# druskus20/volym

Hardware: AMD Instinct MI355X
Metric: Mrays/s + achieved HBM GB/s, 256^3 uint8 @ 1920x1080 (higher is better)
Workload: dtype u8 voxels, f32 compositing

## Files before the change

volym_amd/csrc/raymarch_device.h:

```cpp
#pragma once

#include <hip/hip_runtime.h>

#include "wgsl_math.h"

namespace volym {

enum : uint32_t {
    F_CONE = 1u << 0,
    F_IMP_COLORING = 1u << 1,
    F_OPACITY = 1u << 2,
    F_IMP_RENDERING = 1u << 3,
    F_GAUSSIAN = 1u << 4,
    F_LINEAR = 1u << 5,
    F_WRITE_F32 = 1u << 6,
    F_RASTER = 1u << 7,
};

struct FrameParams {
    float ivp[16];
    float eye[3];
    float thr;
    float base_step;
    float min_step;
// ... 40 lines not shown
#define VOLYM_DF_IN_LDS(fp) (!VOLYM_DEV_SWITCHES || (fp).mc_n <= 32u)
#define VOLYM_DF_LDS_BYTES 16384

enum : uint32_t {
    CULL_CUBE_HULL = 1u << 0,
    CULL_OBJ_HULL = 1u << 1,
    CULL_AABB = 1u << 2,
    CULL_NOTHING_DENSE = 1u << 3,
    CULL_TILE_MASK = 1u << 4,
    CULL_TILE_DEPTH = 1u << 5,
};

struct FrameTables {
    float4 tf_tab[256];
    float4 lut_f[256];
    float ic_alpha[256];
    float rho[256];
};

struct Counters {
    unsigned long long n_vol, n_imp, n_steps, n_dense, n_hit;
};

struct V3 {
    float x, y, z;
};
__device__ __forceinline__ V3 v3(float x, float y, float z) { return V3{x, y, z}; }
__device__ __forceinline__ V3 operator+(V3 a, V3 b) { return v3(a.x + b.x, a.y + b.y, a.z + b.z); }
__device__ __forceinline__ V3 operator-(V3 a, V3 b) { return v3(a.x - b.x, a.y - b.y, a.z - b.z); }
__device__ __forceinline__ V3 operator*(V3 a, float s) { return v3(a.x * s, a.y * s, a.z * s); }
__device__ __forceinline__ V3 operator/(V3 a, float s) { return v3(a.x / s, a.y / s, a.z / s); }
__device__ __forceinline__ float dot_exact(V3 a, V3 b) { return (a.x * b.x + a.y * b.y) + a.z * b.z; }
__device__ __forceinline__ V3 cross(V3 a, V3 b)
{
    return v3(a.y * b.z - a.z * b.y, a.z * b.x - a.x * b.z, a.x * b.y - a.y * b.x);
}
__device__ __forceinline__ float length_exact(V3 a) { return __builtin_sqrtf(dot_exact(a, a)); }
__device__ __forceinline__ V3 normalize_exact(V3 a) { return a / length_exact(a); }
__device__ __forceinline__ float dot_fast(V3 a, V3 b)
{
    return __builtin_fmaf(a.z, b.z, __builtin_fmaf(a.y, b.y, a.x * b.x));
}

__host__ __device__ inline uint32_t brick_count(uint32_t n) { return (n + 3u) >> 2; }

template <bool BRICK>
// ... 510 lines not shown
    r.t_exit = __builtin_fmaxf(exit_, 0.0f);
    r.hit = !(r.t_exit <= r.t_entry);
}

__device__ __forceinline__ Ray make_ray_ieee(const FrameParams& fp, uint32_t gx, uint32_t gy)
{
    Ray r;
    const float scx = static_cast<float>(gx) / static_cast<float>(fp.W);
    const float scy = static_cast<float>(gy) / static_cast<float>(fp.H);
    const float ndx = scx * 2.0f - 1.0f;
    const float ndy = 1.0f - scy * 2.0f;
    float wp[4];
#pragma unroll
    for (int k = 0; k < 4; ++k)
        wp[k] = ((fp.ivp[k] * ndx + fp.ivp[4 + k] * ndy) + fp.ivp[8 + k] * 0.0f) + fp.ivp[12 + k] * 1.0f;
    r.o = v3(fp.eye[0], fp.eye[1], fp.eye[2]);
    const V3 world = v3(wp[0] / wp[3], wp[1] / wp[3], wp[2] / wp[3]);
    r.d = normalize_exact(world - r.o);
    ray_slabs(r, (0.0f - r.o.x) / r.d.x, (1.0f - r.o.x) / r.d.x, (0.0f - r.o.y) / r.d.y, (1.0f - r.o.y) / r.d.y,
              (0.0f - r.o.z) / r.d.z, (1.0f - r.o.z) / r.d.z);
    return r;
}

__device__ __forceinline__ Ray make_ray_shared(const FrameParams& fp, uint32_t gx, uint32_t gy, bool& ok)
{
    Ray r;
    const float scx = div_pixel(static_cast<float>(gx), static_cast<float>(fp.W), fp.rcp_w);
    const float scy = div_pixel(static_cast<float>(gy), static_cast<float>(fp.H), fp.rcp_h);
    const float ndx = scx * 2.0f - 1.0f;
    const float ndy = 1.0f - scy * 2.0f;
    float wp[4];
#pragma unroll
    for (int k = 0; k < 4; ++k)
        wp[k] = ((fp.ivp[k] * ndx + fp.ivp[4 + k] * ndy) + fp.ivp[8 + k] * 0.0f) + fp.ivp[12 + k] * 1.0f;
    r.o = v3(fp.eye[0], fp.eye[1], fp.eye[2]);
    const float rw = rcp_refined(wp[3]);
    const V3 a = v3(div_by(wp[0], wp[3], rw), div_by(wp[1], wp[3], rw), div_by(wp[2], wp[3], rw)) - r.o;
    const float len = length_exact(a);
    const float rl = rcp_refined(len);
    r.d = v3(div_by(a.x, len, rl), div_by(a.y, len, rl), div_by(a.z, len, rl));
    const float rx = rcp_refined(r.d.x), ry = rcp_refined(r.d.y), rz = rcp_refined(r.d.z);
    ray_slabs(r, div_by(0.0f - r.o.x, r.d.x, rx), div_by(1.0f - r.o.x, r.d.x, rx), div_by(0.0f - r.o.y, r.d.y, ry),
              div_by(1.0f - r.o.y, r.d.y, ry), div_by(0.0f - r.o.z, r.d.z, rz), div_by(1.0f - r.o.z, r.d.z, rz));
    const float lo = __builtin_fminf(__builtin_fminf(__builtin_fminf(__builtin_fabsf(wp[0]), __builtin_fabsf(wp[1])), __builtin_fabsf(wp[2])),
                                     __builtin_fminf(__builtin_fabsf(wp[3]), len));
    const float hi = __builtin_fmaxf(__builtin_fmaxf(__builtin_fmaxf(__builtin_fabsf(wp[0]), __builtin_fabsf(wp[1])), __builtin_fabsf(wp[2])),
                                     __builtin_fmaxf(__builtin_fabsf(wp[3]), len));
    const float dlo = __builtin_fminf(__builtin_fminf(__builtin_fabsf(r.d.x), __builtin_fabsf(r.d.y)), __builtin_fabsf(r.d.z));
    ok = lo > fp.setup_lo && hi < 0x1p+40f && dlo > 0x1p-30f;
    return r;
}

template <bool SHARED = true>
__device__ __forceinline__ Ray make_ray(const FrameParams& fp, uint32_t gx, uint32_t gy)
{
    if constexpr (!SHARED) return make_ray_ieee(fp, gx, gy);
    bool ok;
    const Ray r = make_ray_shared(fp, gx, gy, ok);
    if (__builtin_expect(__ballot(!ok) == 0ull, 1)) return r;
    return make_ray_ieee(fp, gx, gy);
}

}
```

volym_amd/csrc/raymarch_pq.h:

```cpp
#pragma once

#include <cstddef>
#include <type_traits>

#include "raymarch_device.h"
#include "worklist_entry.h"

namespace volym {

constexpr int PQ_WAVES = 16;
constexpr int PQ_WAVES_WIDE = 12;
constexpr uint32_t PQ_MIN_LEAP_D = 2;
constexpr int PQ_DP_DEPTH = 2;
constexpr int PQ_ITEMS_LDS = 512;
constexpr int pq_qcap(int k) { return 64 + 64 * k; }
constexpr float PQ_FIX_SCALE = 268435456.0f;
constexpr float PQ_FIX_INV = 1.0f / 268435456.0f;

__device__ __forceinline__ uint32_t lane_rank_in_mask(unsigned long long mask)
{
    return __builtin_amdgcn_mbcnt_hi(static_cast<uint32_t>(mask >> 32), __builtin_amdgcn_mbcnt_lo(static_cast<uint32_t>(mask), 0u));
}

typedef float f32x2 __attribute__((ext_vector_type(2)));
// ... 32 lines not shown
{
    const uint32_t bit = t8y * fp.mask_t8x + t8x;
    return ((fp.tile_mask[bit >> 5] >> (bit & 31u)) & 1u) != 0u;
}
struct PqKernelArgs {
    const uint8_t* vol; const uint8_t* imp; const FrameTables* tables; const uint8_t* df4; const uint2* order; uint32_t n_items; uint16_t* cost;
    uint32_t* out_shard; uint32_t* out_raster; float4* out_f32; Counters* counters; uint4* trace; FrameParams fp;
};
constexpr size_t PQ_FP_KERNARG_OFFSET = offsetof(PqKernelArgs, fp);
static_assert(PQ_FP_KERNARG_OFFSET % 8 == 0 && alignof(FrameParams) == 8, "FrameParams holds pointers: 8-byte aligned in the segment");

template <bool TABLE, bool COUNT, bool TRACE = false, int KSPEC = 1, bool IMP = true, bool BRICK = false, bool IR = false, int WAVES = PQ_WAVES, int CJ = 0, bool LB = false,
          bool RELOAD = true>
__global__ __launch_bounds__(WAVES * 64) void volym_raymarch_pq_kernel(
    const uint8_t* __restrict__ vol, const uint8_t* __restrict__ imp, const FrameTables* __restrict__ tables,
    const uint8_t* __restrict__ df4, const uint2* __restrict__ order, uint32_t n_items, uint16_t* __restrict__ cost,
    uint32_t* __restrict__ out_shard, uint32_t* __restrict__ out_raster, float4* __restrict__ out_f32,
    Counters* __restrict__ counters, uint4* __restrict__ trace, const FrameParams fp)
{
    constexpr int K = TABLE ? KSPEC : 2;
    constexpr int PQ_QCAP = pq_qcap(K);
    static_assert(K <= 4, "the shading queue of K > 4 does not fit the LDS");
    static_assert(CJ == 0 || IR, "look-ahead jobs belong to the importance-rendering instantiation");
    unsigned long long trace_t0 = 0;
    uint32_t trace_iters = 0, trace_flushes = 0, trace_tiles = 0, trace_marched = 0, trace_lanes = 0, trace_accepted = 0, trace_dp_iters = 0;
    unsigned long long tm_leap = 0, tm_samp = 0, tm_flush = 0, tm_mark = 0;
#define PQ_TICK() (TRACE ? __builtin_amdgcn_s_memtime() : 0ull)
    if (TRACE) trace_t0 = __builtin_amdgcn_s_memrealtime();

    __shared__ float4 s_tf_tab[256];
    __shared__ float4 s_lut[TABLE ? 1 : 256];
    __shared__ float s_ic_alpha[256];
    __shared__ float s_rho[256];
    __shared__ __attribute__((aligned(16))) uint8_t s_df[VOLYM_DF_LDS_BYTES];
    constexpr int THREADS = WAVES * 64;
    __shared__ float4 s_q[WAVES][PQ_QCAP];
    __shared__ uint32_t s_qm[WAVES][PQ_QCAP];
    __shared__ float s_qr[TABLE ? 1 : WAVES][TABLE ? 1 : PQ_QCAP];
    __shared__ uint32_t s_acc[WAVES][3][64];
    __shared__ float4 s_hh[WAVES][64];
    __shared__ uint8_t s_mail[(IMP || IR) ? WAVES : 1][(IMP || IR) ? 256 : 1];
    uint8_t (*const s_cres)[(IMP || IR) ? 256 : 1] = s_mail;
    constexpr uint32_t CJ_LPR = CJ == 2 ? 1u : 8u;
    constexpr uint32_t CJ_RPS = 64u / CJ_LPR;
    constexpr uint32_t CJ_CAP = CJ == 2 ? 64u : 32u;
    static_assert(!LB || (TABLE && BRICK && !IMP && !IR && !COUNT && K == 4), "LDS brick staging: bricked layout, common instantiation");
// ... 345 lines not shown
                        const size_t o = static_cast<size_t>(gy) * fe.W + gx;
                        out_raster[o] = packed;
                        if (flags & F_WRITE_F32) out_f32[o] = make_float4(0.0f, 0.0f, 0.0f, tclass == TILE_FILL_MISS ? 1.0f : 0.0f);
                    }
                } else {
                    out_shard[static_cast<size_t>(local_tile) * 256u + sub * 64u + sub_lane] = in_frame ? packed : 0u;
                }
                continue;
            }
        }
        if (TRACE) trace_marched++;

        acc_r[lane] = 0u; acc_g[lane] = 0u; acc_b[lane] = 0u;
        uint32_t q_head = 0, q_count = 0;

        Ray ray;
        ray.o = v3(0.0f, 0.0f, 0.0f); ray.d = v3(0.0f, 0.0f, 0.0f); ray.t_entry = 0.0f; ray.t_exit = 0.0f;
        ray.hit = false;
        if (in_frame) ray = make_ray<TABLE && !IMP && !IR>(fe, gx, gy);
        {
            const V3 hvec = ray_half_vector(ray.d);
            hh[lane] = make_float4(hvec.x, hvec.y, hvec.z, 0.0f);
        }
        bool active = in_frame && ray.hit;
        if (COUNT && active) n_hit++;
        float t = active ? ray.t_entry : 0.0f, cur = base, acc_a = active ? 0.0f : 1.0f;
        bool last_dense = false;
        if (culling && tclass == TILE_HIT_TEST) active = false;
        float t_end = ray.t_exit;
        if (culling && (fe.cull & CULL_AABB) && active) {
            const float rx = __builtin_amdgcn_rcpf(ray.d.x), ry = __builtin_amdgcn_rcpf(ray.d.y), rz = __builtin_amdgcn_rcpf(ray.d.z);
            const float ax0 = (fe.aabb_lo[0] - ray.o.x) * rx, ax1 = (fe.aabb_hi[0] - ray.o.x) * rx;
            const float ay0 = (fe.aabb_lo[1] - ray.o.y) * ry, ay1 = (fe.aabb_hi[1] - ray.o.y) * ry;
            const float az0 = (fe.aabb_lo[2] - ray.o.z) * rz, az1 = (fe.aabb_hi[2] - ray.o.z) * rz;
            float tn = __builtin_fmaxf(__builtin_fmaxf(__builtin_fminf(ax0, ax1), __builtin_fminf(ay0, ay1)), __builtin_fminf(az0, az1));
            float tf = __builtin_fminf(__builtin_fminf(__builtin_fmaxf(ax0, ax1), __builtin_fmaxf(ay0, ay1)), __builtin_fmaxf(az0, az1));
            tn = tn - 2.0e-5f * __builtin_fabsf(tn) - 1.0e-6f;
            tf = tf + 2.0e-5f * __builtin_fabsf(tf) + 1.0e-6f;
            if (fe.cull & CULL_TILE_DEPTH) {
                const auto* td = (const __attribute__((address_space(4))) uint32_t*)fe.tile_depth;
                const uint32_t t8 = (ty * 2u + (sub >> 1)) * fe.mask_t8x + tx * 2u + (sub & 1u);
                tn = __builtin_fmaxf(tn, __uint_as_float(~td[t8]));
                tf = __builtin_fminf(tf, __uint_as_float(td[32u * fe.mask_words + t8]));
            }
            const bool outside_static = (ray.d.x == 0.0f && (ray.o.x < fe.aabb_lo[0] || ray.o.x > fe.aabb_hi[0])) ||
                                        (ray.d.y == 0.0f && (ray.o.y < fe.aabb_lo[1] || ray.o.y > fe.aabb_hi[1])) ||
                                        (ray.d.z == 0.0f && (ray.o.z < fe.aabb_lo[2] || ray.o.z > fe.aabb_hi[2]));
            if (outside_static || !(tn <= tf)) {
                active = false;
            } else {
                t_end = __builtin_fminf(t_end, tf);
                const float t_first = __builtin_fminf(tn, t_end);
// ... 43 lines not shown
                    grad = v3(static_cast<float>(bxp - bxm), static_cast<float>(byp - bym), static_cast<float>(bzp - bzm));
                } else {
                    grad = v3(sample_density(g, s_rho, linear, v3(pos.x + o, pos.y, pos.z)) -
                                  sample_density(g, s_rho, linear, v3(pos.x - o, pos.y, pos.z)),
                              sample_density(g, s_rho, linear, v3(pos.x, pos.y + o, pos.z)) -
                                  sample_density(g, s_rho, linear, v3(pos.x, pos.y - o, pos.z)),
                              sample_density(g, s_rho, linear, v3(pos.x, pos.y, pos.z + o)) -
                                  sample_density(g, s_rho, linear, v3(pos.x, pos.y, pos.z - o)));
                }
                const float4 hv = hh[owner];
                const V3 shaded = blinn_phong_h(color, grad, v3(hv.x, hv.y, hv.z));
                atomicAdd(&acc_r[owner], static_cast<uint32_t>(__builtin_fmaf(shaded.x * w, PQ_FIX_SCALE, 0.5f)));
                atomicAdd(&acc_g[owner], static_cast<uint32_t>(__builtin_fmaf(shaded.y * w, PQ_FIX_SCALE, 0.5f)));
                atomicAdd(&acc_b[owner], static_cast<uint32_t>(__builtin_fmaf(shaded.z * w, PQ_FIX_SCALE, 0.5f)));
            }
            q_head += n;
            if (q_head >= PQ_QCAP) q_head -= PQ_QCAP;
            q_count -= n;
            __builtin_amdgcn_fence(__ATOMIC_SEQ_CST, "wavefront");
            __builtin_amdgcn_wave_barrier();
            if (TRACE) tm_flush += PQ_TICK() - fl0;
        };

        auto append = [&](bool emit, V3 p, float w, uint32_t meta, float rho) __attribute__((always_inline)) {
            if (VOLYM_DEV_SWITCHES && (fp.dev & 128u)) return;
            const unsigned long long mask = __ballot(emit);
            if (mask == 0ull) return;
            if (emit) {
                const uint32_t e0 = q_head + q_count + lane_rank_in_mask(mask), e = min(e0, e0 - PQ_QCAP);
                q4[e] = make_float4(p.x, p.y, p.z, w); qm[e] = meta;
                if (!TABLE) qr[e] = rho;
            }
            q_count += static_cast<uint32_t>(__popcll(mask));
            if (!TABLE && q_count >= 64u) flush(64u);
        };
        auto drain = [&]() __attribute__((always_inline)) { while (q_count >= 64u) flush(64u); };

        if (VOLYM_DEV_SWITCHES && (fp.dev & 256u)) active = false;
        if (TRACE) tm_mark = PQ_TICK();
        bool leap_ok = true;
        auto leap_phase = [&]() __attribute__((always_inline)) {
            active = active && t < t_end && acc_a < 0.95f;
            const bool want_leap = active && !last_dense && leap_ok;
            if (__ballot(want_leap) != 0ull) {
                const V3 pos = ray.o + ray.d * t;
                const float cxf = __builtin_floorf(pos.x * mcf), cyf = __builtin_floorf(pos.y * mcf), czf = __builtin_floorf(pos.z * mcf);
                const int cx = static_cast<int>(cxf), cy = static_cast<int>(cyf), cz = static_cast<int>(czf);
                const bool in_range = static_cast<uint32_t>(cx | cy | cz) < fp.mc_n;
                const uint32_t ci = in_range ? mad_u24(mad_u24(static_cast<uint32_t>(cz), fp.mc_n, static_cast<uint32_t>(cy)), fp.mc_n, static_cast<uint32_t>(cx)) : 0u;
                uint32_t D = (static_cast<uint32_t>(VOLYM_DF_IN_LDS(fp) ? s_df[ci >> 1] : df4[ci >> 1]) >> ((ci & 1u) * 4u)) & 15u;
                if (!(want_leap && in_range)) D = 0u;
                if (D >= PQ_MIN_LEAP_D) {
                    const float eps = gauss ? 4.0e-5f + 0.0101f : 4.0e-5f;
                    const float a = static_cast<float>(D - 1u) * inv_mc - eps;
                    const float lx = __builtin_fmaf(cxf, inv_mc, -a), hx = __builtin_fmaf(cxf, inv_mc, a + inv_mc);
                    const float ly = __builtin_fmaf(cyf, inv_mc, -a), hy = __builtin_fmaf(cyf, inv_mc, a + inv_mc);
                    const float lz = __builtin_fmaf(czf, inv_mc, -a), hz = __builtin_fmaf(czf, inv_mc, a + inv_mc);
                    const float ex = __builtin_fmaxf(__builtin_fmaf(lx, idx_, nox), __builtin_fmaf(hx, idx_, nox));
                    const float ey = __builtin_fmaxf(__builtin_fmaf(ly, idy_, noy), __builtin_fmaf(hy, idy_, noy));
                    const float ez = __builtin_fmaxf(__builtin_fmaf(lz, idz_, noz), __builtin_fmaf(hz, idz_, noz));
                    float te = __builtin_fminf(__builtin_fminf(ex, ey), ez);
                    te = te - 2.0e-5f * __builtin_fabsf(te);
                    const float t_stop = __builtin_fminf(te, t_end);
                    if (!COUNT) {
                        while (cur < base && t < t_stop) {
                            cur = __builtin_fminf(base, cur * 1.5f);
                            t += cur;
                        }
                        tile_trips++;
                        replay_saturated(t, t_stop, base);
                    }
                    while (COUNT && t < t_stop) {
                        if (COUNT) {
                            n_steps++; n_imp++;
                            if (gauss) {
                                const V3 q = ray.o + ray.d * t;
                                for (int i = -2; i <= 2; ++i) if (!outside01(q + ray.d * (static_cast<float>(i) * 0.005f))) n_vol++;
                            } else {
                                n_vol++;
                            }
                        }
                        cur = __builtin_fminf(base, cur * 1.5f);
                        t += cur;
                    }
                    if (!(t < t_end)) active = false;
                }
            }

        };

        if (dp) {
            const uint32_t kq = lane & 3u, qsh = lane & 60u;
            if constexpr (!IMP) {
                constexpr int J = PQ_DP_DEPTH;
                bool try_leap = true;
                active = active && t < t_end;
                while (__ballot(active) != 0ull) {
                    tile_iters++;
                    if (TRACE) { trace_iters++; trace_dp_iters++; trace_lanes += static_cast<uint32_t>(__popcll(__ballot(active))); tm_mark = PQ_TICK(); }
                    if (try_leap && !(VOLYM_DEV_SWITCHES && (fp.dev & 2u))) leap_phase();
                    if (TRACE) { const unsigned long long now = PQ_TICK(); tm_leap += now - tm_mark; tm_mark = now; }
                    constexpr int N = 4 * J;
                    float ts[N], cb[N], my_t[J];
                    {
                        float tt = t, cc = cur;
#pragma unroll
                        for (int sidx = 0; sidx < N; ++sidx) {
                            ts[sidx] = tt; cb[sidx] = cc;
                            if ((sidx & 3) == 0) my_t[sidx >> 2] = tt;
                            else my_t[sidx >> 2] = kq == static_cast<uint32_t>(sidx & 3) ? tt : my_t[sidx >> 2];
                            cc = last_dense ? min_step : __builtin_fminf(base, cc * 1.5f);
                            tt += cc;
                        }
                    }
                    V3 my_pos[J];
                    uint32_t my_b[J], my_ib[J];
#pragma unroll
                    for (int j = 0; j < J; ++j) {
                        my_ib[j] = 255u;
                        my_pos[j] = ray.o + ray.d * my_t[j];
                        const uint32_t off_j = nearest_offset(g, my_pos[j]);
                        my_b[j] = vol[off_j];
                        if (IR) my_ib[j] = imp[off_j];
                    }
                    drain();
                    uint32_t cm = 0;
                    float a4[J][4];
#pragma unroll
                    for (int j = 0; j < J; ++j) {
                        cm |= (static_cast<uint32_t>(__ballot(my_b[j] >= fp.thr_byte) >> qsh) & 15u) << (4 * j);
                        const int a_bits = __float_as_int(s_tf_tab[my_b[j]].w);
                        a4[j][0] = __int_as_float(__builtin_amdgcn_mov_dpp(a_bits, 0x00, 0xf, 0xf, true));
                        a4[j][1] = __int_as_float(__builtin_amdgcn_mov_dpp(a_bits, 0x55, 0xf, 0xf, true));
                        a4[j][2] = __int_as_float(__builtin_amdgcn_mov_dpp(a_bits, 0xaa, 0xf, 0xf, true));
                        a4[j][3] = __int_as_float(__builtin_amdgcn_mov_dpp(a_bits, 0xff, 0xf, 0xf, true));
                    }
                    uint32_t sm = 0;
                    if (IR) {
                        bool need[J], ahead[J];
#pragma unroll
                        for (int j = 0; j < J; ++j) { need[j] = active && my_b[j] >= fp.thr_byte && my_ib[j] < 255u; ahead[j] = false; }
                        if constexpr (CJ != 0) {
                            cj_lookahead(need, my_t, ray.o, ray.d, ray.t_exit, ahead);
                        } else if (flags & F_CONE) {
#pragma unroll
                            for (int j = 0; j < J; ++j)
                                ahead[j] = ahead_cone_wave(g, fp_here(), need[j], my_pos[j], ray.d, ray.t_exit, lane, fp.cone_cos[lane & 7u] * 0.2f, fp.cone_sin[lane & 7u] * 0.2f);
                        } else {
                            bool any_need = false;
#pragma unroll
                            for (int j = 0; j < J; ++j) any_need = any_need || need[j];
                            if (__ballot(any_need) != 0ull) ahead_straight_wave<J>(g, fp_here(), need, my_t, ray.o, ray.d, ray.t_exit, lane, mail, ahead, &la_rounds);
                        }
#pragma unroll
                        for (int j = 0; j < J; ++j) sm |= (static_cast<uint32_t>(__ballot(need[j] && ahead[j]) >> qsh) & 15u) << (4 * j);
                    }
                    uint32_t n_t = 0, n_a = 0;
                    float a_run = acc_a, a_after[N], my_w[J];
#pragma unroll
                    for (int sidx = 0; sidx < N; ++sidx) {
                        n_t += ts[sidx] < t_end ? 1u : 0u;
                        n_a += a_run < 0.95f ? 1u : 0u;
                        const float w = (1.0f - a_run) * a4[sidx >> 2][sidx & 3];
                        if ((sidx & 3) == 0) my_w[sidx >> 2] = w;
                        else my_w[sidx >> 2] = kq == static_cast<uint32_t>(sidx & 3) ? w : my_w[sidx >> 2];
                        a_run = (((cm & ~sm) >> sidx) & 1u) ? a_run + w : a_run;
                        a_after[sidx] = a_run;
                    }
                    const uint32_t full = (1u << N) - 1u;
                    const uint32_t mism = cm ^ (last_dense ? full : 0u);
                    const uint32_t n_c = min(static_cast<uint32_t>(__builtin_ctz(mism | (1u << N))) + 1u, static_cast<uint32_t>(N));
                    const uint32_t n_acc = min(min(n_t, n_a), n_c);
                    const uint32_t em = active ? (cm & ~sm & ((1u << n_acc) - 1u)) : 0u;
                    bool my_emit[J];
#pragma unroll
                    for (int j = 0; j < J; ++j) my_emit[j] = ((em >> (4 * j + kq)) & 1u) != 0u;
                    if (TRACE && kq == 0u && active) trace_accepted += n_acc;
                    const uint32_t last = n_acc - 1u;
                    float t_sel = ts[0], cb_sel = cb[0], a_sel = a_after[0];
#pragma unroll
                    for (int sidx = 1; sidx < N; ++sidx) {
                        const bool ge = last >= static_cast<uint32_t>(sidx);
                        t_sel = ge ? ts[sidx] : t_sel; cb_sel = ge ? cb[sidx] : cb_sel; a_sel = ge ? a_after[sidx] : a_sel;
                    }
                    const bool dl = ((cm >> last) & 1u) != 0u;
                    const bool last_dense_before = last_dense;
                    const float cur_new = dl ? min_step : __builtin_fminf(base, cb_sel * 1.5f);
                    if (active) {
                        cur = cur_new;
                        t = t_sel + cur_new;
                        acc_a = a_sel;
                        last_dense = dl;
                    }
                    leap_ok = !dl && !last_dense_before && n_acc == static_cast<uint32_t>(N);
                    try_leap = __ballot(active && leap_ok) != 0ull;
                    active = active && t < t_end && acc_a < 0.95f;
#pragma unroll
                    for (int j = 0; j < J; ++j) append(my_emit[j], my_pos[j], my_w[j], own | (my_b[j] << 8), 0.0f);
                    if (TRACE) tm_samp += PQ_TICK() - tm_mark;
                }
            } else {
            const bool use_alpha_dp = imp_coloring || (flags & F_OPACITY) != 0u;
            while (__ballot(active) != 0ull) {
                tile_iters++;
                if (TRACE) { trace_iters++; trace_dp_iters++; trace_lanes += static_cast<uint32_t>(__popcll(__ballot(active))); tm_mark = PQ_TICK(); }
                leap_phase();
                if (TRACE) { const unsigned long long now = PQ_TICK(); tm_leap += now - tm_mark; tm_mark = now; }
                float ts4[4], cs4[4];
                {
                    float tt = t, cc = cur;
#pragma unroll
                    for (int j = 0; j < 4; ++j) {
                        ts4[j] = tt;
                        cc = last_dense ? min_step : __builtin_fminf(base, cc * 1.5f);
                        cs4[j] = cc;
                        tt += cc;
                    }
                }
                const float tk = kq == 0u ? ts4[0] : (kq == 1u ? ts4[1] : (kq == 2u ? ts4[2] : ts4[3]));
                const V3 pos = ray.o + ray.d * tk;
                const uint32_t off = nearest_offset(g, pos);
// ... 52 lines not shown
                                        alpha += w;
                                    } else {
                                        if (static_cast<uint32_t>(j) == kq) { my_w = 1.0f; my_emit = true; }
                                        alpha = 1.0f;
                                        done = true; finished = true;
                                    }
                                }
                                if (dj != last_dense) done = true;
                            }
                        }
                    }
                    if (TRACE && kq == 0u) trace_accepted += static_cast<uint32_t>(last + 1);
                    if (last >= 0) {
                        const bool dl = ((quad_d >> last) & 1u) != 0u;
                        const float cur_before = last == 0 ? cur : (last == 1 ? cs4[0] : (last == 2 ? cs4[1] : cs4[2]));
                        const float t_last = last == 0 ? ts4[0] : (last == 1 ? ts4[1] : (last == 2 ? ts4[2] : ts4[3]));
                        cur = dl ? min_step : __builtin_fminf(base, cur_before * 1.5f);
                        if (!(finished && !use_alpha_dp && dl)) t = t_last + cur;
                        last_dense = dl;
                    }
                    acc_a = alpha;
                    if (finished) active = false;
                }
                append(my_emit, pos, my_w, own | (b << 8) | (ib << 16), rho_k);
                if (TRACE) tm_samp += PQ_TICK() - tm_mark;
            }
            }
        } else {
        while (__ballot(active) != 0ull) {
            tile_iters++;
            if (TRACE) { trace_iters++; trace_lanes += static_cast<uint32_t>(__popcll(__ballot(active))); tm_mark = PQ_TICK(); if (active) trace_ray_iters++; }
            leap_phase();
            if (TRACE) { const unsigned long long now = PQ_TICK(); tm_leap += now - tm_mark; tm_mark = now; }
            float ts[K];
            uint32_t offs[K], bs[K], ibs[K];
            float rhos[K];
            uint32_t taps[K];
            {
                float tt = t, cc = cur;
#pragma unroll
                for (int k = 0; k < K; ++k) {
                    ts[k] = tt;
                    cc = last_dense ? min_step : __builtin_fminf(base, cc * 1.5f);
                    tt += cc;
                }
                if constexpr (K % 2 == 0) {
#pragma unroll
                    for (int k = 0; k < K; k += 2) {
                        const f32x2 tp = {ts[k], ts[k + 1]};
                        const f32x2 ux = (ray.o.x + ray.d.x * tp) * g.fnx, uy = (ray.o.y + ray.d.y * tp) * g.fny, uz = (ray.o.z + ray.d.z * tp) * g.fnz;
                        offs[k] = voxel_offset(g, clamp_texel(floor_to_int(ux.x), static_cast<int>(g.hix)), clamp_texel(floor_to_int(uy.x), static_cast<int>(g.hiy)),
                                               clamp_texel(floor_to_int(uz.x), static_cast<int>(g.hiz)));
                        offs[k + 1] = voxel_offset(g, clamp_texel(floor_to_int(ux.y), static_cast<int>(g.hix)), clamp_texel(floor_to_int(uy.y), static_cast<int>(g.hiy)),
                                                   clamp_texel(floor_to_int(uz.y), static_cast<int>(g.hiz)));
                    }
                } else {
#pragma unroll
                    for (int k = 0; k < K; ++k) offs[k] = nearest_offset(g, ray.o + ray.d * ts[k]);
                }
#pragma unroll
                for (int k = 0; k < K; ++k) {
                    bs[k] = 0; ibs[k] = 0; rhos[k] = 0.0f; taps[k] = 1;
                    if (TABLE && !LB) bs[k] = vol[offs[k]];
                    if (IR) ibs[k] = imp[offs[k]];
                    if (active) {
                        if (!IR && need_imp) ibs[k] = imp[offs[k]];
                        if (!TABLE) {
                            const V3 p = ray.o + ray.d * ts[k];
                            uint32_t cnt = 0;
                            if (gauss) rhos[k] = sample_density_smoothed<true>(g, s_rho, linear, fp, p, ray.d, cnt);
                            else { rhos[k] = sample_density(g, s_rho, linear, p); cnt = 1; }
                            taps[k] = cnt;
                        }
                    }
                }
            }

            uint32_t lb_slots = 0xffffffffu;
            uint32_t lb_ld[2] = {0u, 0u}, lb_dst = 0xffffu;
            if constexpr (LB) {
                const uint32_t* const vol32 = reinterpret_cast<const uint32_t*>(vol);
                const unsigned long long act = __ballot(active);
                uint32_t used = 0u, n_new = 0u, lb_b[2] = {0u, 0u};
#pragma unroll
                for (int k = 0; k < K; ++k) {
                    const uint32_t bk = offs[k] >> 6;
                    unsigned long long todo = act;
                    while (todo != 0ull) {
                        const uint32_t b = __builtin_amdgcn_readlane(bk, __builtin_ctzll(todo));
                        const unsigned long long same = __ballot(bk == b) & todo;
                        todo &= ~same;
                        const uint32_t hit = static_cast<uint32_t>(__ballot(lb_tag == b)) & ((1u << LB_SLOTS) - 1u);
                        uint32_t sl;
                        if (hit != 0u) {
                            sl = static_cast<uint32_t>(__builtin_ctz(hit));
                            if (VOLYM_DEV_SWITCHES && (fp.dev & 512u) && lane == 0u) atomicAdd(&counters->n_hit, 1ull);
                        } else {
                            const uint32_t free_places = ~used & ((1u << LB_SLOTS) - 1u);
                            if (free_places == 0u || n_new == 8u) {
                                if (VOLYM_DEV_SWITCHES && (fp.dev & 512u) && lane == 0u) atomicAdd(&counters->n_dense, 1ull);
                                continue;
                            }
                            const uint32_t from_next = free_places & ~((1u << lb_next) - 1u);
                            sl = static_cast<uint32_t>(__builtin_ctz(from_next != 0u ? from_next : free_places));
                            lb_next = (sl + 1u) & (LB_SLOTS - 1u);
// ... 14 lines not shown
                if ((lb_dst >> 8) != 0xffu) lb_ld[1] = vol32[lb_b[1] * 16u + (lane & 15u)];
#pragma unroll
                for (int k = 0; k < K; ++k)
                    if (active && ((lb_slots >> (8 * k)) & 0xffu) == 0xffu) bs[k] = vol[offs[k]];
            }

            if (TABLE) drain();
            if constexpr (LB) {
                uint32_t* const lbw = s_lb[wave];
                if ((lb_dst & 0xffu) != 0xffu) lbw[(lb_dst & 0xffu) * 16u + (lane & 15u)] = lb_ld[0];
                if ((lb_dst >> 8) != 0xffu) lbw[(lb_dst >> 8) * 16u + (lane & 15u)] = lb_ld[1];
                const uint8_t* const lbb = reinterpret_cast<const uint8_t*>(lbw);
#pragma unroll
                for (int k = 0; k < K; ++k) {
                    const uint32_t sl = (lb_slots >> (8 * k)) & 0xffu;
                    if (sl != 0xffu) bs[k] = lbb[sl * 64u + (offs[k] & 63u)];
                }
            }

            if constexpr (TABLE && !COUNT && !IMP) {
                float a_tab[K];
#pragma unroll
                for (int k = 0; k < K; ++k) a_tab[k] = s_tf_tab[bs[k]].w;
                const bool predicted = last_dense;
                bool supp[K];
#pragma unroll
                for (int k = 0; k < K; ++k) supp[k] = false;
                if (IR) {
                    bool need[K];
                    bool chain = active;
#pragma unroll
                    for (int k = 0; k < K; ++k) {
                        const bool dense_k = bs[k] >= fp.thr_byte;
                        need[k] = chain && dense_k && ibs[k] < 255u;
                        chain = chain && dense_k == predicted;
                    }
                    if constexpr (CJ != 0) {
                        cj_lookahead(need, ts, ray.o, ray.d, ray.t_exit, supp);
                    } else if (flags & F_CONE) {
#pragma unroll
                        for (int k = 0; k < K; ++k)
                            supp[k] = ahead_cone_wave(g, fp_here(), need[k], ray.o + ray.d * ts[k], ray.d, ray.t_exit, lane, fp.cone_cos[lane & 7u] * 0.2f, fp.cone_sin[lane & 7u] * 0.2f);
                    } else {
                        bool any_need = false;
#pragma unroll
                        for (int k = 0; k < K; ++k) any_need = any_need || need[k];
                        if (__ballot(any_need) != 0ull) ahead_straight_wave<K>(g, fp_here(), need, ts, ray.o, ray.d, ray.t_exit, lane, mail, supp, &la_rounds);
                    }
#pragma unroll
                    for (int k = 0; k < K; ++k) supp[k] = supp[k] && need[k];
                }
                bool valid = active;
#pragma unroll
                for (int k = 0; k < K; ++k) {
                    const bool go = valid && t < t_end && acc_a < 0.95f;
                    if (TRACE && go) trace_accepted++;
                    const bool dense = bs[k] >= fp.thr_byte;
                    const bool emit = go && dense && !supp[k];
                    const float w = (1.0f - acc_a) * a_tab[k];
                    const V3 pos = ray.o + ray.d * t;
                    acc_a = emit ? acc_a + w : acc_a;
                    const float cur_next = dense ? min_step : __builtin_fminf(base, cur * 1.5f);
                    cur = go ? cur_next : cur;
                    t = go ? t + cur_next : t;
                    last_dense = go ? dense : last_dense;
                    valid = go && dense == predicted;
                    if (k == K - 1) leap_ok = go && !dense && !predicted;
                    append(emit, pos, w, own | (bs[k] << 8), 0.0f);
                }
                active = active && t < t_end && acc_a < 0.95f;
                if (TRACE) tm_samp += PQ_TICK() - tm_mark;
                continue;
            }
            bool ahead_pre[K];
            constexpr bool PRE_AHEAD = IMP && !COUNT && K > 1;
            const bool pre_ahead = PRE_AHEAD && imp_rendering && !imp_coloring;
            if (PRE_AHEAD && pre_ahead && (flags & F_CONE)) {
                bool chain = active;
#pragma unroll
                for (int k = 0; k < K; ++k) {
                    const bool dense_k = TABLE ? bs[k] >= fp.thr_byte : rhos[k] >= thr;
                    const bool need_k = chain && dense_k && ibs[k] < 255u;
                    chain = chain && dense_k == last_dense;
                    ahead_pre[k] = ahead_cone_wave(g, fp_here(), need_k, ray.o + ray.d * ts[k], ray.d, ray.t_exit, lane, fp.cone_cos[lane & 7u] * 0.2f, fp.cone_sin[lane & 7u] * 0.2f);
                }
            } else if (PRE_AHEAD && pre_ahead) {
                bool need[K];
                bool chain = active;
#pragma unroll
                for (int k = 0; k < K; ++k) {
                    const bool dense_k = TABLE ? bs[k] >= fp.thr_byte : rhos[k] >= thr;
                    need[k] = chain && dense_k && ibs[k] < 255u;
                    chain = chain && dense_k == last_dense;
// ... 40 lines not shown
                                                              : ahead_straight<COUNT>(g, fp, pos, ray.d, ray.t_exit, n_imp);
                                suppressed = ibs[k] < 255u && ahead;
                            }
                            if (TABLE) alpha_step = s_tf_tab[bs[k]].w;
                            else alpha_step = 1.0f - wgsl_pow(1.0f - sample_tf(s_lut, fp.tf_n, rhos[k]).w, fp.alpha_y);
                        }
                        if (!suppressed) {
                            if (COUNT) n_vol += 6;
                            emit = true;
                            if (use_alpha) {
                                w = (1.0f - acc_a) * alpha_step;
                                acc_a += w;
                            } else {
                                w = 1.0f;
                                acc_a = 1.0f;
                                advance = false;
                                active = false;
                                valid = false;
                            }
                        }
                    }
                    if (advance) t += cur;
                }
                append(emit, pos, w, own | (bs[k] << 8) | (ibs[k] << 16), rhos[k]);
            }
            if (TRACE) tm_samp += PQ_TICK() - tm_mark;
        }
        }
        drain();
        if (q_count) flush(q_count);

        if (in_frame && (!dp || (lane & 3u) == 0u)) {
            const float out_r = static_cast<float>(acc_r[own]) * PQ_FIX_INV, out_g = static_cast<float>(acc_g[own]) * PQ_FIX_INV,
                        out_b = static_cast<float>(acc_b[own]) * PQ_FIX_INV;
            const uint32_t packed = pack_rgba8(out_r, out_g, out_b, acc_a);
            if (flags & F_RASTER) {
                const size_t o = static_cast<size_t>(gy) * fe.W + gx;
                out_raster[o] = packed;
                if (flags & F_WRITE_F32) out_f32[o] = TRACE ? make_float4(static_cast<float>(trace_ray_iters), static_cast<float>(tile_iters), out_b, acc_a) : make_float4(out_r, out_g, out_b, acc_a);
            } else {
                out_shard[static_cast<size_t>(local_tile) * 256u + sub * 64u + sub_lane] = packed;
            }
        } else if (!in_frame && !(flags & F_RASTER) && (!dp || (lane & 3u) == 0u)) {
            out_shard[static_cast<size_t>(local_tile) * 256u + sub * 64u + sub_lane] = 0u;
        }
#ifndef VOLYM_COST_FLUSH
#define VOLYM_COST_FLUSH 2u
// ... 59 lines not shown
```

Measured before the change: 87790.

## Carry ray-march lane state as wave-wide ballot masks instead of per-lane bools

Replaces per-lane boolean control state (active, last_dense, leap_ok, emit, suppression) with 64-bit wave lane masks built by ballot and read back through inverse ballot. Loop conditions and the queue append then use the mask directly, so the repeated ballots on loop exits and emit decisions go away and the state can sit in scalar registers. A MASKS specialisation is added for table-mode, uninstrumented, non-importance instantiations, including a mask-based AABB and tile-depth cull. It adds a parallel code path that must keep matching the bool semantics, and some mask updates now differ subtly, for example the first-step go check.

```diff
diff --git a/volym_amd/csrc/raymarch_device.h b/volym_amd/csrc/raymarch_device.h
--- a/volym_amd/csrc/raymarch_device.h
+++ b/volym_amd/csrc/raymarch_device.h
@@ -86,6 +86,10 @@
     unsigned long long n_vol, n_imp, n_steps, n_dense, n_hit;
 };
 
+typedef unsigned long long lanemask;
+__device__ __forceinline__ lanemask lanes_where(bool single_compare) { return __builtin_amdgcn_ballot_w64(single_compare); }
+__device__ __forceinline__ bool lane_of(lanemask m) { return __builtin_amdgcn_inverse_ballot_w64(m); }
+
 struct V3 {
     float x, y, z;
 };
@@ -642,7 +646,7 @@
     return r;
 }
 
-__device__ __forceinline__ Ray make_ray_shared(const FrameParams& fp, uint32_t gx, uint32_t gy, bool& ok)
+__device__ __forceinline__ Ray make_ray_shared(const FrameParams& fp, uint32_t gx, uint32_t gy, lanemask& m_ok)
 {
     Ray r;
     const float scx = div_pixel(static_cast<float>(gx), static_cast<float>(fp.W), fp.rcp_w);
@@ -667,7 +671,14 @@
     const float hi = __builtin_fmaxf(__builtin_fmaxf(__builtin_fmaxf(__builtin_fabsf(wp[0]), __builtin_fabsf(wp[1])), __builtin_fabsf(wp[2])),
                                      __builtin_fmaxf(__builtin_fabsf(wp[3]), len));
     const float dlo = __builtin_fminf(__builtin_fminf(__builtin_fabsf(r.d.x), __builtin_fabsf(r.d.y)), __builtin_fabsf(r.d.z));
-    ok = lo > fp.setup_lo && hi < 0x1p+40f && dlo > 0x1p-30f;
+    m_ok = lanes_where(lo > fp.setup_lo) & lanes_where(hi < 0x1p+40f) & lanes_where(dlo > 0x1p-30f);
+    return r;
+}
+__device__ __forceinline__ Ray make_ray_shared(const FrameParams& fp, uint32_t gx, uint32_t gy, bool& ok)
+{
+    lanemask m_ok;
+    const Ray r = make_ray_shared(fp, gx, gy, m_ok);
+    ok = lane_of(m_ok);
     return r;
 }
 
@@ -675,9 +686,9 @@
 __device__ __forceinline__ Ray make_ray(const FrameParams& fp, uint32_t gx, uint32_t gy)
 {
     if constexpr (!SHARED) return make_ray_ieee(fp, gx, gy);
-    bool ok;
-    const Ray r = make_ray_shared(fp, gx, gy, ok);
-    if (__builtin_expect(__ballot(!ok) == 0ull, 1)) return r;
+    lanemask m_ok;
+    const Ray r = make_ray_shared(fp, gx, gy, m_ok);
+    if (__builtin_expect((~m_ok & lanes_where(true)) == 0ull, 1)) return r;
     return make_ray_ieee(fp, gx, gy);
 }
 
diff --git a/volym_amd/csrc/raymarch_pq.h b/volym_amd/csrc/raymarch_pq.h
--- a/volym_amd/csrc/raymarch_pq.h
+++ b/volym_amd/csrc/raymarch_pq.h
@@ -78,6 +78,8 @@
     constexpr int PQ_QCAP = pq_qcap(K);
     static_assert(K <= 4, "the shading queue of K > 4 does not fit the LDS");
     static_assert(CJ == 0 || IR, "look-ahead jobs belong to the importance-rendering instantiation");
+    constexpr bool MASKS = TABLE && !COUNT && !IMP;
+    static_assert(IMP || MASKS, "the pinned-flag instantiations are table mode and uninstrumented");
     unsigned long long trace_t0 = 0;
     uint32_t trace_iters = 0, trace_flushes = 0, trace_tiles = 0, trace_marched = 0, trace_lanes = 0, trace_accepted = 0, trace_dp_iters = 0;
     unsigned long long tm_leap = 0, tm_samp = 0, tm_flush = 0, tm_mark = 0;
@@ -469,12 +471,41 @@
             const V3 hvec = ray_half_vector(ray.d);
             hh[lane] = make_float4(hvec.x, hvec.y, hvec.z, 0.0f);
         }
-        bool active = in_frame && ray.hit;
+        lanemask m_active = lanes_where(gx < fe.W) & lanes_where(gy < fe.H) & lanes_where(!(ray.t_exit <= ray.t_entry));
+        lanemask m_last = 0ull, m_leap_ok = ~0ull;
+        bool active = MASKS ? lane_of(m_active) : in_frame && ray.hit;
         if (COUNT && active) n_hit++;
         float t = active ? ray.t_entry : 0.0f, cur = base, acc_a = active ? 0.0f : 1.0f;
         bool last_dense = false;
-        if (culling && tclass == TILE_HIT_TEST) active = false;
+        if (culling && tclass == TILE_HIT_TEST) { active = false; m_active = 0ull; }
         float t_end = ray.t_exit;
+        if constexpr (MASKS) {
+            if (culling && (fe.cull & CULL_AABB) && m_active != 0ull) {
+                const float rx = __builtin_amdgcn_rcpf(ray.d.x), ry = __builtin_amdgcn_rcpf(ray.d.y), rz = __builtin_amdgcn_rcpf(ray.d.z);
+                const float ax0 = (fe.aabb_lo[0] - ray.o.x) * rx, ax1 = (fe.aabb_hi[0] - ray.o.x) * rx;
+                const float ay0 = (fe.aabb_lo[1] - ray.o.y) * ry, ay1 = (fe.aabb_hi[1] - ray.o.y) * ry;
+                const float az0 = (fe.aabb_lo[2] - ray.o.z) * rz, az1 = (fe.aabb_hi[2] - ray.o.z) * rz;
+                float tn = __builtin_fmaxf(__builtin_fmaxf(__builtin_fminf(ax0, ax1), __builtin_fminf(ay0, ay1)), __builtin_fminf(az0, az1));
+                float tf = __builtin_fminf(__builtin_fminf(__builtin_fmaxf(ax0, ax1), __builtin_fmaxf(ay0, ay1)), __builtin_fmaxf(az0, az1));
+                tn = tn - 2.0e-5f * __builtin_fabsf(tn) - 1.0e-6f;
+                tf = tf + 2.0e-5f * __builtin_fabsf(tf) + 1.0e-6f;
+                if (fe.cull & CULL_TILE_DEPTH) {
+                    const auto* td = (const __attribute__((address_space(4))) uint32_t*)fe.tile_depth;
+                    const uint32_t t8 = (ty * 2u + (sub >> 1)) * fe.mask_t8x + tx * 2u + (sub & 1u);
+                    tn = __builtin_fmaxf(tn, __uint_as_float(~td[t8]));
+                    tf = __builtin_fminf(tf, __uint_as_float(td[32u * fe.mask_words + t8]));
+                }
+                const lanemask m_static = (lanes_where(ray.d.x == 0.0f) & (lanes_where(ray.o.x < fe.aabb_lo[0]) | lanes_where(ray.o.x > fe.aabb_hi[0]))) |
+                                          (lanes_where(ray.d.y == 0.0f) & (lanes_where(ray.o.y < fe.aabb_lo[1]) | lanes_where(ray.o.y > fe.aabb_hi[1]))) |
+                                          (lanes_where(ray.d.z == 0.0f) & (lanes_where(ray.o.z < fe.aabb_lo[2]) | lanes_where(ray.o.z > fe.aabb_hi[2])));
+                m_active &= ~m_static & lanes_where(tn <= tf);
+                if (lane_of(m_active)) {
+                    t_end = __builtin_fminf(t_end, tf);
+                    const float t_first = __builtin_fminf(tn, t_end);
+                    replay_saturated(t, t_first, base);
+                }
+            }
+        } else
         if (culling && (fe.cull & CULL_AABB) && active) {
             const float rx = __builtin_amdgcn_rcpf(ray.d.x), ry = __builtin_amdgcn_rcpf(ray.d.y), rz = __builtin_amdgcn_rcpf(ray.d.z);
             const float ax0 = (fe.aabb_lo[0] - ray.o.x) * rx, ax1 = (fe.aabb_hi[0] - ray.o.x) * rx;
@@ -564,11 +595,10 @@
             if (TRACE) tm_flush += PQ_TICK() - fl0;
         };
 
-        auto append = [&](bool emit, V3 p, float w, uint32_t meta, float rho) __attribute__((always_inline)) {
+        auto append = [&](lanemask mask, V3 p, float w, uint32_t meta, float rho) __attribute__((always_inline)) {
             if (VOLYM_DEV_SWITCHES && (fp.dev & 128u)) return;
-            const unsigned long long mask = __ballot(emit);
-            if (mask == 0ull) return;
-            if (emit) {
+            if constexpr (!MASKS) if (mask == 0ull) return;
+            if (lane_of(mask)) {
                 const uint32_t e0 = q_head + q_count + lane_rank_in_mask(mask), e = min(e0, e0 - PQ_QCAP);
                 q4[e] = make_float4(p.x, p.y, p.z, w); qm[e] = meta;
                 if (!TABLE) qr[e] = rho;
@@ -578,20 +608,29 @@
         };
         auto drain = [&]() __attribute__((always_inline)) { while (q_count >= 64u) flush(64u); };
 
-        if (VOLYM_DEV_SWITCHES && (fp.dev & 256u)) active = false;
+        if (VOLYM_DEV_SWITCHES && (fp.dev & 256u)) { active = false; m_active = 0ull; }
         if (TRACE) tm_mark = PQ_TICK();
         bool leap_ok = true;
         auto leap_phase = [&]() __attribute__((always_inline)) {
-            active = active && t < t_end && acc_a < 0.95f;
-            const bool want_leap = active && !last_dense && leap_ok;
-            if (__ballot(want_leap) != 0ull) {
+            bool want_leap = false;
+            lanemask m_want = 0ull;
+            if constexpr (MASKS) {
+                m_active &= lanes_where(t < t_end) & lanes_where(acc_a < 0.95f);
+                m_want = m_active & ~m_last & m_leap_ok;
+            } else {
+                active = active && t < t_end && acc_a < 0.95f;
+                want_leap = active && !last_dense && leap_ok;
+                m_want = __ballot(want_leap);
+            }
+            if (m_want != 0ull) {
                 const V3 pos = ray.o + ray.d * t;
                 const float cxf = __builtin_floorf(pos.x * mcf), cyf = __builtin_floorf(pos.y * mcf), czf = __builtin_floorf(pos.z * mcf);
                 const int cx = static_cast<int>(cxf), cy = static_cast<int>(cyf), cz = static_cast<int>(czf);
                 const bool in_range = static_cast<uint32_t>(cx | cy | cz) < fp.mc_n;
+                if constexpr (MASKS) want_leap = lane_of(m_want & lanes_where(static_cast<uint32_t>(cx | cy | cz) < fp.mc_n));
                 const uint32_t ci = in_range ? mad_u24(mad_u24(static_cast<uint32_t>(cz), fp.mc_n, static_cast<uint32_t>(cy)), fp.mc_n, static_cast<uint32_t>(cx)) : 0u;
                 uint32_t D = (static_cast<uint32_t>(VOLYM_DF_IN_LDS(fp) ? s_df[ci >> 1] : df4[ci >> 1]) >> ((ci & 1u) * 4u)) & 15u;
-                if (!(want_leap && in_range)) D = 0u;
+                if (!(MASKS ? want_leap : want_leap && in_range)) D = 0u;
                 if (D >= PQ_MIN_LEAP_D) {
                     const float eps = gauss ? 4.0e-5f + 0.0101f : 4.0e-5f;
                     const float a = static_cast<float>(D - 1u) * inv_mc - eps;
@@ -625,8 +664,9 @@
                         cur = __builtin_fminf(base, cur * 1.5f);
                         t += cur;
                     }
-                    if (!(t < t_end)) active = false;
-                }
+                    if (!MASKS && !(t < t_end)) active = false;
+                }
+                if constexpr (MASKS) m_active &= lanes_where(t < t_end);
             }
 
         };
@@ -636,10 +676,10 @@
             if constexpr (!IMP) {
                 constexpr int J = PQ_DP_DEPTH;
                 bool try_leap = true;
-                active = active && t < t_end;
-                while (__ballot(active) != 0ull) {
+                m_active &= lanes_where(t < t_end);
+                while (m_active != 0ull) {
                     tile_iters++;
-                    if (TRACE) { trace_iters++; trace_dp_iters++; trace_lanes += static_cast<uint32_t>(__popcll(__ballot(active))); tm_mark = PQ_TICK(); }
+                    if (TRACE) { trace_iters++; trace_dp_iters++; trace_lanes += static_cast<uint32_t>(__popcll(m_active)); tm_mark = PQ_TICK(); }
                     if (try_leap && !(VOLYM_DEV_SWITCHES && (fp.dev & 2u))) leap_phase();
                     if (TRACE) { const unsigned long long now = PQ_TICK(); tm_leap += now - tm_mark; tm_mark = now; }
                     constexpr int N = 4 * J;
@@ -651,7 +691,7 @@
                             ts[sidx] = tt; cb[sidx] = cc;
                             if ((sidx & 3) == 0) my_t[sidx >> 2] = tt;
                             else my_t[sidx >> 2] = kq == static_cast<uint32_t>(sidx & 3) ? tt : my_t[sidx >> 2];
-                            cc = last_dense ? min_step : __builtin_fminf(base, cc * 1.5f);
+                            cc = lane_of(m_last) ? min_step : __builtin_fminf(base, cc * 1.5f);
                             tt += cc;
                         }
                     }
@@ -680,8 +720,13 @@
                     uint32_t sm = 0;
                     if (IR) {
                         bool need[J], ahead[J];
-#pragma unroll
-                        for (int j = 0; j < J; ++j) { need[j] = active && my_b[j] >= fp.thr_byte && my_ib[j] < 255u; ahead[j] = false; }
+                        lanemask m_need[J], m_any_need = 0ull;
+#pragma unroll
+                        for (int j = 0; j < J; ++j) {
+                            m_need[j] = m_active & lanes_where(my_b[j] >= fp.thr_byte) & lanes_where(my_ib[j] < 255u);
+                            m_any_need |= m_need[j];
+                            need[j] = lane_of(m_need[j]); ahead[j] = false;
+                        }
                         if constexpr (CJ != 0) {
                             cj_lookahead(need, my_t, ray.o, ray.d, ray.t_exit, ahead);
                         } else if (flags & F_CONE) {
@@ -689,13 +734,10 @@
                             for (int j = 0; j < J; ++j)
                                 ahead[j] = ahead_cone_wave(g, fp_here(), need[j], my_pos[j], ray.d, ray.t_exit, lane, fp.cone_cos[lane & 7u] * 0.2f, fp.cone_sin[lane & 7u] * 0.2f);
                         } else {
-                            bool any_need = false;
-#pragma unroll
-                            for (int j = 0; j < J; ++j) any_need = any_need || need[j];
-                            if (__ballot(any_need) != 0ull) ahead_straight_wave<J>(g, fp_here(), need, my_t, ray.o, ray.d, ray.t_exit, lane, mail, ahead, &la_rounds);
+                            if (m_any_need != 0ull) ahead_straight_wave<J>(g, fp_here(), need, my_t, ray.o, ray.d, ray.t_exit, lane, mail, ahead, &la_rounds);
                         }
 #pragma unroll
-                        for (int j = 0; j < J; ++j) sm |= (static_cast<uint32_t>(__ballot(need[j] && ahead[j]) >> qsh) & 15u) << (4 * j);
+                        for (int j = 0; j < J; ++j) sm |= (static_cast<uint32_t>((m_need[j] & __ballot(ahead[j])) >> qsh) & 15u) << (4 * j);
                     }
                     uint32_t n_t = 0, n_a = 0;
                     float a_run = acc_a, a_after[N], my_w[J];
@@ -710,14 +752,14 @@
                         a_after[sidx] = a_run;
                     }
                     const uint32_t full = (1u << N) - 1u;
-                    const uint32_t mism = cm ^ (last_dense ? full : 0u);
+                    const uint32_t mism = cm ^ (lane_of(m_last) ? full : 0u);
                     const uint32_t n_c = min(static_cast<uint32_t>(__builtin_ctz(mism | (1u << N))) + 1u, static_cast<uint32_t>(N));
                     const uint32_t n_acc = min(min(n_t, n_a), n_c);
-                    const uint32_t em = active ? (cm & ~sm & ((1u << n_acc) - 1u)) : 0u;
-                    bool my_emit[J];
-#pragma unroll
-                    for (int j = 0; j < J; ++j) my_emit[j] = ((em >> (4 * j + kq)) & 1u) != 0u;
-                    if (TRACE && kq == 0u && active) trace_accepted += n_acc;
+                    const uint32_t em = cm & ~sm & ((1u << n_acc) - 1u);
+                    lanemask m_emit[J];
+#pragma unroll
+                    for (int j = 0; j < J; ++j) m_emit[j] = m_active & lanes_where(((em >> (4 * j + kq)) & 1u) != 0u);
+                    if (TRACE && kq == 0u && lane_of(m_active)) trace_accepted += n_acc;
                     const uint32_t last = n_acc - 1u;
                     float t_sel = ts[0], cb_sel = cb[0], a_sel = a_after[0];
 #pragma unroll
@@ -725,20 +767,19 @@
                         const bool ge = last >= static_cast<uint32_t>(sidx);
                         t_sel = ge ? ts[sidx] : t_sel; cb_sel = ge ? cb[sidx] : cb_sel; a_sel = ge ? a_after[sidx] : a_sel;
                     }
-                    const bool dl = ((cm >> last) & 1u) != 0u;
-                    const bool last_dense_before = last_dense;
-                    const float cur_new = dl ? min_step : __builtin_fminf(base, cb_sel * 1.5f);
-                    if (active) {
+                    const lanemask m_dl = lanes_where(((cm >> last) & 1u) != 0u);
+                    const float cur_new = lane_of(m_dl) ? min_step : __builtin_fminf(base, cb_sel * 1.5f);
+                    if (lane_of(m_active)) {
                         cur = cur_new;
                         t = t_sel + cur_new;
                         acc_a = a_sel;
-                        last_dense = dl;
-                    }
-                    leap_ok = !dl && !last_dense_before && n_acc == static_cast<uint32_t>(N);
-                    try_leap = __ballot(active && leap_ok) != 0ull;
-                    active = active && t < t_end && acc_a < 0.95f;
-#pragma unroll
-                    for (int j = 0; j < J; ++j) append(my_emit[j], my_pos[j], my_w[j], own | (my_b[j] << 8), 0.0f);
+                    }
+                    m_leap_ok = ~m_dl & ~m_last & lanes_where(n_acc == static_cast<uint32_t>(N));
+                    m_last = (m_active & m_dl) | (~m_active & m_last);
+                    try_leap = (m_active & m_leap_ok) != 0ull;
+                    m_active &= lanes_where(t < t_end) & lanes_where(acc_a < 0.95f);
+#pragma unroll
+                    for (int j = 0; j < J; ++j) append(m_emit[j], my_pos[j], my_w[j], own | (my_b[j] << 8), 0.0f);
                     if (TRACE) tm_samp += PQ_TICK() - tm_mark;
                 }
             } else {
@@ -837,14 +878,15 @@
                     acc_a = alpha;
                     if (finished) active = false;
                 }
-                append(my_emit, pos, my_w, own | (b << 8) | (ib << 16), rho_k);
+                append(__ballot(my_emit), pos, my_w, own | (b << 8) | (ib << 16), rho_k);
                 if (TRACE) tm_samp += PQ_TICK() - tm_mark;
             }
             }
         } else {
-        while (__ballot(active) != 0ull) {
+        while ((MASKS ? m_active : __ballot(active)) != 0ull) {
+            if constexpr (MASKS) active = lane_of(m_active);
             tile_iters++;
-            if (TRACE) { trace_iters++; trace_lanes += static_cast<uint32_t>(__popcll(__ballot(active))); tm_mark = PQ_TICK(); if (active) trace_ray_iters++; }
+            if (TRACE) { trace_iters++; trace_lanes += static_cast<uint32_t>(__popcll(MASKS ? m_active : __ballot(active))); tm_mark = PQ_TICK(); if (active) trace_ray_iters++; }
             leap_phase();
             if (TRACE) { const unsigned long long now = PQ_TICK(); tm_leap += now - tm_mark; tm_mark = now; }
             float ts[K];
@@ -856,7 +898,7 @@
 #pragma unroll
                 for (int k = 0; k < K; ++k) {
                     ts[k] = tt;
-                    cc = last_dense ? min_step : __builtin_fminf(base, cc * 1.5f);
+                    cc = (MASKS ? lane_of(m_last) : last_dense) ? min_step : __builtin_fminf(base, cc * 1.5f);
                     tt += cc;
                 }
                 if constexpr (K % 2 == 0) {
@@ -878,7 +920,7 @@
                     bs[k] = 0; ibs[k] = 0; rhos[k] = 0.0f; taps[k] = 1;
                     if (TABLE && !LB) bs[k] = vol[offs[k]];
                     if (IR) ibs[k] = imp[offs[k]];
-                    if (active) {
+                    if constexpr (!MASKS) if (active) {
                         if (!IR && need_imp) ibs[k] = imp[offs[k]];
                         if (!TABLE) {
                             const V3 p = ray.o + ray.d * ts[k];
@@ -895,7 +937,8 @@
             uint32_t lb_ld[2] = {0u, 0u}, lb_dst = 0xffffu;
             if constexpr (LB) {
                 const uint32_t* const vol32 = reinterpret_cast<const uint32_t*>(vol);
-                const unsigned long long act = __ballot(active);
+                const unsigned long long act = m_active;
+                if constexpr (MASKS) active = lane_of(m_active);
                 uint32_t used = 0u, n_new = 0u, lb_b[2] = {0u, 0u};
 #pragma unroll
                 for (int k = 0; k < K; ++k) {
@@ -956,18 +999,21 @@
                 float a_tab[K];
 #pragma unroll
                 for (int k = 0; k < K; ++k) a_tab[k] = s_tf_tab[bs[k]].w;
-                const bool predicted = last_dense;
-                bool supp[K];
-#pragma unroll
-                for (int k = 0; k < K; ++k) supp[k] = false;
+                const lanemask m_predicted = m_last;
+                lanemask m_supp[K];
+#pragma unroll
+                for (int k = 0; k < K; ++k) m_supp[k] = 0ull;
                 if (IR) {
-                    bool need[K];
-                    bool chain = active;
+                    bool need[K], supp[K];
+                    lanemask m_need[K], m_any_need = 0ull;
+                    lanemask m_chain = m_active;
 #pragma unroll
                     for (int k = 0; k < K; ++k) {
-                        const bool dense_k = bs[k] >= fp.thr_byte;
-                        need[k] = chain && dense_k && ibs[k] < 255u;
-                        chain = chain && dense_k == predicted;
+                        const lanemask m_dense_k = lanes_where(bs[k] >= fp.thr_byte);
+                        m_need[k] = m_chain & m_dense_k & lanes_where(ibs[k] < 255u);
+                        m_chain &= ~(m_dense_k ^ m_predicted);
+                        m_any_need |= m_need[k];
+                        need[k] = lane_of(m_need[k]); supp[k] = false;
                     }
                     if constexpr (CJ != 0) {
                         cj_lookahead(need, ts, ray.o, ray.d, ray.t_exit, supp);
@@ -976,33 +1022,31 @@
                         for (int k = 0; k < K; ++k)
                             supp[k] = ahead_cone_wave(g, fp_here(), need[k], ray.o + ray.d * ts[k], ray.d, ray.t_exit, lane, fp.cone_cos[lane & 7u] * 0.2f, fp.cone_sin[lane & 7u] * 0.2f);
                     } else {
-                        bool any_need = false;
-#pragma unroll
-                        for (int k = 0; k < K; ++k) any_need = any_need || need[k];
-                        if (__ballot(any_need) != 0ull) ahead_straight_wave<K>(g, fp_here(), need, ts, ray.o, ray.d, ray.t_exit, lane, mail, supp, &la_rounds);
-                    }
-#pragma unroll
-                    for (int k = 0; k < K; ++k) supp[k] = supp[k] && need[k];
-                }
-                bool valid = active;
+                        if (m_any_need != 0ull) ahead_straight_wave<K>(g, fp_here(), need, ts, ray.o, ray.d, ray.t_exit, lane, mail, supp, &la_rounds);
+                    }
+#pragma unroll
+                    for (int k = 0; k < K; ++k) m_supp[k] = m_need[k] & __ballot(supp[k]);
+                }
+                lanemask m_valid = m_active;
 #pragma unroll
                 for (int k = 0; k < K; ++k) {
-                    const bool go = valid && t < t_end && acc_a < 0.95f;
+                    const lanemask m_go = k == 0 ? m_valid : m_valid & lanes_where(t < t_end) & lanes_where(acc_a < 0.95f);
+                    const lanemask m_dense = lanes_where(bs[k] >= fp.thr_byte);
+                    const lanemask m_emit = m_go & m_dense & ~m_supp[k];
+                    const bool go = lane_of(m_go);
                     if (TRACE && go) trace_accepted++;
-                    const bool dense = bs[k] >= fp.thr_byte;
-                    const bool emit = go && dense && !supp[k];
                     const float w = (1.0f - acc_a) * a_tab[k];
                     const V3 pos = ray.o + ray.d * t;
-                    acc_a = emit ? acc_a + w : acc_a;
-                    const float cur_next = dense ? min_step : __builtin_fminf(base, cur * 1.5f);
+                    acc_a = lane_of(m_emit) ? acc_a + w : acc_a;
+                    const float cur_next = lane_of(m_dense) ? min_step : __builtin_fminf(base, cur * 1.5f);
                     cur = go ? cur_next : cur;
                     t = go ? t + cur_next : t;
-                    last_dense = go ? dense : last_dense;
-                    valid = go && dense == predicted;
-                    if (k == K - 1) leap_ok = go && !dense && !predicted;
-                    append(emit, pos, w, own | (bs[k] << 8), 0.0f);
-                }
-                active = active && t < t_end && acc_a < 0.95f;
+                    m_last = (m_go & m_dense) | (~m_go & m_last);
+                    m_valid = m_go & ~(m_dense ^ m_predicted);
+                    if (k == K - 1) m_leap_ok = m_go & ~m_dense & ~m_predicted;
+                    append(m_emit, pos, w, own | (bs[k] << 8), 0.0f);
+                }
+                m_active &= lanes_where(t < t_end) & lanes_where(acc_a < 0.95f);
                 if (TRACE) tm_samp += PQ_TICK() - tm_mark;
                 continue;
             }
@@ -1089,7 +1133,7 @@
                     }
                     if (advance) t += cur;
                 }
-                append(emit, pos, w, own | (bs[k] << 8) | (ibs[k] << 16), rhos[k]);
+                append(__ballot(emit), pos, w, own | (bs[k] << 8) | (ibs[k] << 16), rhos[k]);
             }
             if (TRACE) tm_samp += PQ_TICK() - tm_mark;
         }
```

Measured after the change: 90600, median of 6. 3.2% higher.
